# alexncoleman/WeaklySupervisedDL

Hardware: AMD Instinct MI355X
Metric: SegmentationModel train img/s at B=16 256x256 (higher is better)
Workload: dtype f32

## Files before the change

weaklysuperviseddl_amd/csrc/conv_igemm.hip:

```cpp
#include "common.h"

#include <type_traits>
#include <algorithm>
#include <cstdint>
#include <mutex>

typedef float f32x16 __attribute__((ext_vector_type(16)));

namespace {

constexpr int kThreads = 256;

struct ConvSrc {
    const float* x;
    const float* wt;
    const float* x_amax;
    int KH, KW, bh, ch, K, Cin;
    long long x_bs;
    unsigned x_bytes;
};

struct ConvP {
    const float* x;
    const float* wt;
    float* y;
    const float* scale;
    const float* shift;
    const float* res;
    int B, Cin, H, W, Cout, OH, OW, KH, KW;
    int ah, bh, ch, sh;
    int K;
    long long x_bs, y_bs, res_bs;
    int relu, accumulate;
    int P;
    unsigned x_bytes;
    int ksplit;
    float* slab;
    int ow0, own;
    int nb;
    int b_ow0[4], b_own[4], b_tile0[5];
    int grid_x;
    int xcd_py;
    int xcd_rowfast;
    int tile_img_major;
    const float* x_amax;
    float* y_amax;
    const uint8_t* acc_mask;
    const float* acc_base;
    int nsrc;
    ConvSrc src[3];
};

__device__ __forceinline__ float acc_prev(const ConvP& p, const float* ptr) {
    float o = *ptr;
    if (p.acc_mask) {
        const long long e = ptr - p.acc_base;
        if (!((p.acc_mask[e >> 3] >> (e & 7)) & 1)) o = 0.f;
    }
    return o;
}

template <int BM, int BN, int WM, bool ALIGNED>
__global__ __launch_bounds__(kThreads) void conv_igemm_kernel(ConvP p) {
    constexpr int BK = 16;
    constexpr int WN = 4 / WM;
    constexpr int MI = BM / WM / 32;
    constexpr int NI = BN / WN / 32;
    static_assert(MI >= 1 && NI >= 1 && MI * 32 * WM == BM && NI * 32 * WN == BN, "bad tile");
    constexpr int A_F4 = BK * BM / 4 / kThreads;
    constexpr int B_STEP = kThreads / BN;
    constexpr int B_PER = BK / B_STEP;

    __shared__ float As[2][BK * BM];
    __shared__ float Bs[2][BK * BN];
    __shared__ int vtaps[64];
    constexpr int kTab = ALIGNED ? 1 : 1024;
    __shared__ int ktab[kTab][2];
// ... 1149 lines not shown
    WSDL_LAUNCH_CHECK();
    return WSDL_OK;
}

wsdl::Opt g_conv_split{1};
wsdl::Opt g_conv_arith{1};
bool split_eligible(int rows, int kc, int T) {
    return g_conv_split && kc % 16 == 0 && T <= 9 && split_layout_bytes(g_conv_arith, (long long)T * kc, rows) < (1ll << 31);
}

wsdl::Opt g_xcd_map{1};
int choose_xcd_py(const ConvP& p, int gx, int gy) {
    if (!g_xcd_map || p.ksplit > 1 || ((long long)gx * gy) % 8 != 0) return 0;
    const double wb = (g_conv_arith ? 4.0 : 6.0) * (double)p.K * p.Cout, xb = 4.0 * (double)p.B * p.Cin * p.H * p.W;
    int best = 0;
    double best_cost = 0.0;
    for (int py = 1; py <= 8; py *= 2) {
        const int px = 8 / py;
        if (gy % py || gx % px) continue;
        if (g_xcd_map > 10 && py != g_xcd_map - 10) continue;
        const double cost = wb * px + xb * py;
        if (!best || cost < best_cost) { best = py; best_cost = cost; }
    }
    if (g_xcd_map == 1 && (best <= 1 || best_cost > 0.9 * (wb * 8 + xb))) return 0;
    return best;
}

template <int BM, int BN, int WM, int BK>
int launch_split(const ConvP& p_in, hipStream_t s, dim3 grid) {
    ConvP p = p_in;
    grid.z = p.ksplit > 1 ? p.ksplit : 1;
    p.xcd_py = choose_xcd_py(p, grid.x, grid.y);
    p.tile_img_major = 0;
    constexpr bool MF = BK == 32;
    WSDL_TRACE("split<%d,%d,%d> ar=%d %s ks=%d xcd_py=%d nb=%d grid=%ux%ux%u", BM, BN, BK, (int)g_conv_arith,
               (MF && g_conv_arith) ? "mfma16x16x32" : "mfma32x32x16", p.ksplit, p.xcd_py, p.nb, grid.x, grid.y, grid.z);
    if (g_conv_arith == 2)
        hipLaunchKernelGGL((conv_igemm_split_kernel<BM, BN, WM, BK, kThreads, 2, MF>), grid, dim3(kThreads), 0, s, p);
    else if (g_conv_arith)
        hipLaunchKernelGGL((conv_igemm_split_kernel<BM, BN, WM, BK, kThreads, 1, MF>), grid, dim3(kThreads), 0, s, p);
    else
        hipLaunchKernelGGL((conv_igemm_split_kernel<BM, BN, WM, BK, kThreads, 0>), grid, dim3(kThreads), 0, s, p);
    WSDL_LAUNCH_CHECK();
    return WSDL_OK;
}

wsdl::Opt g_conv_il{1};
int launch_split_256x128(const ConvP& p_in, hipStream_t s) {
    ConvP p = p_in;
    dim3 grid(p.grid_x > 0 ? p.grid_x : wsdl::cdiv(p.P, 128), wsdl::cdiv(p.Cout, 256), p.ksplit > 1 ? p.ksplit : 1);
    p.xcd_py = choose_xcd_py(p, grid.x, grid.y);
    p.xcd_rowfast = 0;
    p.tile_img_major = 0;
    if (p.nsrc > 0 && grid.y % 2 == 0 && ((long long)grid.x * grid.y) % 8 == 0) {
        int py = 4;
        while (py > 1 && (grid.y % py || grid.x % (8 / py))) py /= 2;
        if (grid.y % py == 0 && grid.x % (8 / py) == 0) {
            p.xcd_py = py;
            p.xcd_rowfast = 1;
        }
    }
    WSDL_TRACE("split<256,128,16> ar=%d il=%d nsrc=%d ks=%d xcd_py=%d rowfast=%d imgmajor=%d nb=%d grid=%ux%ux%u", (int)g_conv_arith,
               (int)(g_conv_arith == 1 && g_conv_il), p.nsrc, p.ksplit, p.xcd_py, p.xcd_rowfast, p.tile_img_major, p.nb, grid.x, grid.y, grid.z);
    if (p.nsrc > 0) {
        if (g_conv_arith == 2) hipLaunchKernelGGL((conv_igemm_split_kernel<256, 128, 4, 16, 512, 2, false, true>), grid, dim3(512), 0, s, p);
        else if (g_conv_arith && g_conv_il)
            hipLaunchKernelGGL((conv_igemm_split_kernel<256, 128, 4, 16, 512, 1, false, true, true>), grid, dim3(512), 0, s, p);
        else if (g_conv_arith) hipLaunchKernelGGL((conv_igemm_split_kernel<256, 128, 4, 16, 512, 1, false, true>), grid, dim3(512), 0, s, p);
        else hipLaunchKernelGGL((conv_igemm_split_kernel<256, 128, 4, 16, 512, 0, false, true>), grid, dim3(512), 0, s, p);
        WSDL_LAUNCH_CHECK();
        return WSDL_OK;
    }
    if (g_conv_arith == 2) hipLaunchKernelGGL((conv_igemm_split_kernel<256, 128, 4, 16, 512, 2>), grid, dim3(512), 0, s, p);
    else if (g_conv_arith && g_conv_il)
        hipLaunchKernelGGL((conv_igemm_split_kernel<256, 128, 4, 16, 512, 1, false, false, true>), grid, dim3(512), 0, s, p);
    else if (g_conv_arith) hipLaunchKernelGGL((conv_igemm_split_kernel<256, 128, 4, 16, 512, 1>), grid, dim3(512), 0, s, p);
    else hipLaunchKernelGGL((conv_igemm_split_kernel<256, 128, 4, 16, 512, 0>), grid, dim3(512), 0, s, p);
    WSDL_LAUNCH_CHECK();
    return WSDL_OK;
}

template <int BM, int BN, int WM>
int launch_cfg(const ConvP& p, hipStream_t s, bool aligned, bool split) {
    dim3 grid(p.grid_x > 0 ? p.grid_x : wsdl::cdiv(p.P, BN), wsdl::cdiv(p.Cout, BM));
    constexpr bool kSmallTile = BM * BN <= 128 * 64;
    if (split) {
        if constexpr (kSmallTile) {
            if (p.Cin % 32 == 0) {
                return launch_split<BM, BN, WM, 32>(p, s, grid);
            }
        }
        return launch_split<BM, BN, WM, 16>(p, s, grid);
    } else if (aligned) {
        if constexpr (kSmallTile) {
            if (p.Cin % 32 == 0) {
                return launch_fast<BM, BN, WM, 32>(p, s, grid);
// ... 387 lines not shown
            hipLaunchKernelGGL(wgrad_reduce_kernel, dim3(d.nblocks), dim3(256), 0, s, d.slab, d.dw, d.S, d.Cout, d.Cin, d.T, d.accumulate,
                               d.live);
            break;
    }
    WSDL_LAUNCH_CHECK();
    return WSDL_OK;
}

template <int BM, int BN, int WM>
int launch_wgrad_fast(const WgradP& p, hipStream_t s, int S) {
    dim3 grid(p.N / BN, p.Cout / BM, S);
    hipLaunchKernelGGL((conv_wgrad_fast_kernel<BM, BN, WM, 16>), grid, dim3(kThreads), 2 * (BM + BN) * 17 * sizeof(float), s, p);
    WSDL_LAUNCH_CHECK();
    return WSDL_OK;
}

}

extern "C" {

int wsdl_set_option(const char* name, int value) {
    WSDL_REQUIRE(name, "set_option: null name");
    static std::mutex mu;
    std::lock_guard<std::mutex> lock(mu);
    WSDL_REQUIRE(wsdl::g_plans_recording.load() == 0,
                 "set_option(%s): a launch plan is being recorded (its launches are chosen under ONE option set)", name);
    if (!strcmp(name, "tile_threshold")) { g_tile_threshold = value; return WSDL_OK; }
    if (!strcmp(name, "conv_split")) { g_conv_split = value != 0; return WSDL_OK; }
    if (!strcmp(name, "stem_kernel")) { g_stem_kernel = value != 0; return WSDL_OK; }
    if (!strcmp(name, "wgrad_direct")) { g_wgrad_direct = value; return WSDL_OK; }
    if (!strcmp(name, "wgrad_chan_scale")) { g_wgrad_chan_scale = value != 0; return WSDL_OK; }
    if (!strcmp(name, "wgrad_dyraw")) { g_wgrad_dyraw = value; return WSDL_OK; }
    if (!strcmp(name, "conv_il")) { g_conv_il = value != 0; return WSDL_OK; }
    if (!strcmp(name, "xcd_map")) { g_xcd_map = value; return WSDL_OK; }
    if (!strcmp(name, "ksplit_target")) { g_ksplit_target = value; return WSDL_OK; }
    if (!strcmp(name, "ksplit_max")) { g_ksplit_max = value; return WSDL_OK; }
    if (!strcmp(name, "ksplit_min_chunks")) { g_ksplit_min_chunks = value > 0 ? value : 1; return WSDL_OK; }
    if (!strcmp(name, "conv_arith")) {
        WSDL_REQUIRE(value >= 0 && value <= 2, "conv_arith: 0 (bf16x3), 1 (fp16x2), 2 (fp16x2, low piece at 2^11)");
        g_conv_arith = value;
        return WSDL_OK;
    }
    if (!strcmp(name, "range_sentinel")) { wsdl::g_range_sentinel = value != 0; return WSDL_OK; }
    if (!strcmp(name, "group_tps10")) { g_group_tps10 = value > 0 ? value : 45; return WSDL_OK; }
    if (!strcmp(name, "bn_resident")) { wsdl::g_bn_resident = value; return WSDL_OK; }
    if (!strcmp(name, "bn_wide_c")) { wsdl::g_bn_wide_c = value; return WSDL_OK; }
    if (!strcmp(name, "layercam_tail_mod")) {
        WSDL_REQUIRE(value >= 0 && value <= 32, "layercam_tail_mod: 0..32");
        wsdl::g_layercam_tail_mod = value;
        return WSDL_OK;
    }
    if (!strcmp(name, "wgrad_split")) { g_wgrad_split = value != 0; return WSDL_OK; }
    if (!strcmp(name, "wgrad_xcd")) { g_wgrad_xcd = value; return WSDL_OK; }
    if (!strcmp(name, "wgrad_min_tiles")) { g_wgrad_min_tiles = value > 0 ? value : 1; return WSDL_OK; }
    if (!strcmp(name, "wgrad_blocks")) { g_wgrad_blocks = value > 0 ? value : 768; return WSDL_OK; }
    wsdl::set_error("set_option: unknown option %s", name);
    return WSDL_EINVAL;
}

size_t wsdl_conv2d_weight_layout_bytes(int Cout, int Cin, int kh, int kw, int dgrad, int* is_plain) {
    const int T = kh * kw;
    const bool split = dgrad ? split_eligible(Cin, Cout, T) : split_eligible(Cout, Cin, T);
    if (is_plain) *is_plain = split ? 0 : 1;
    const size_t n = (size_t)Cout * Cin * T;
    return split ? (size_t)split_layout_bytes(g_conv_arith, (long long)T * (dgrad ? Cout : Cin), dgrad ? Cin : Cout) : n * 4;
}
// ... 159 lines not shown
        p.B = B; p.Cin = Cin; p.H = H; p.W = W; p.Cout = Cout; p.OH = H; p.OW = W; p.KH = p.KW = k[i];
        p.ah = 1; p.bh = dil[i]; p.ch = -pad; p.sh = 1;
        p.K = k[i] * k[i] * Cin;
        p.x_bs = xbs;
        p.y_bs = (y_bs && y_bs[i]) ? y_bs[i] : (long long)Cout * H * W;
        p.res_bs = p.y_bs;
        WSDL_REQUIRE(p.x_bs >= (long long)Cin * H * W && p.y_bs >= (long long)Cout * H * W, "conv2d_fwd_group: batch stride smaller than an image");
        p.P = B * H * W;
        p.x_bytes = (unsigned)(((long long)(B - 1) * p.x_bs + (long long)Cin * H * W) * 4);
        p.x_amax = x_amax;
        p.ow0 = 0; p.own = W; p.nb = 1;
        Band bands[8];
        int nb = 1;
        bands[0] = Band{0, W};
        nb = column_bands(W, W, p.ah, p.bh, p.ch, p.sh, p.KW, bands);
        int tiles = 0;
        for (int b = 0; b < nb && nb > 1; ++b) {
            p.b_ow0[b] = bands[b].ow0;
            p.b_own[b] = bands[b].own;
            p.b_tile0[b] = tiles;
            tiles += wsdl::cdiv((long long)B * H * bands[b].own, 128);
        }
        p.nb = nb;
        p.b_tile0[nb > 1 ? nb : 0] = tiles;
        const int gx = nb > 1 ? tiles : wsdl::cdiv(p.P, 128), gy = Cout / 256;
        const int ks = group_ksplit(group_max_taps(H, W, k[i], dil[i]));
        p.ksplit = ks;
        if (ks > 1) {
            p.slab = reinterpret_cast<float*>(wsp);
            wsp += wsdl::align_up((size_t)ks * Cout * p.P * sizeof(float), 256);
        }
        p.xcd_py = (start % 8 == 0) ? choose_xcd_py(p, gx, gy) : 0;
        p.tile_img_major = k[i] > 1;
        grp.start[j] = start;
        grp.gx[j] = gx;
        grp.gy[j] = gy;
        start += gx * gy * ks;
        const double f = 2.0 * p.P * (double)Cout * p.K;
        flops += f;
        if (wsdl::prof_enabled()) {
            for (int b = 0; b < nb; ++b) {
                ConvP q = p;
                q.ow0 = bands[b].ow0; q.own = bands[b].own; q.P = B * H * q.own;
                executed += f * ((double)q.own / W) * igemm_executed_fraction(q, 128);
            }
        }
        bytes += 4.0 * ((double)p.K * Cout + (double)p.P * Cout);
    }
    grp.start[n] = start;
    {
        int ns = 0;
        bool same = true;
        for (int j = 0; j < n; ++j) {
            ns += grp.p[j].ksplit;
            same = same && grp.gx[j] * grp.gy[j] == grp.gx[0] * grp.gy[0];
        }
        if (same && ns <= 8 && (8 % ns == 0)) {
            grp.ns = ns;
            int s = 0;
            for (int j = 0; j < n; ++j)
                for (int z = 0; z < grp.p[j].ksplit; ++z) {
                    grp.s_prob[s] = j;
                    grp.s_slice[s] = z;
                    ++s;
                }
            for (int j = 0; j < n; ++j) grp.p[j].xcd_py = 0;
        }
    }
    {
        wsdl::ProfScope prof(WSDL_PROF_SPLIT_GROUP, s, flops, wsdl::prof_enabled() ? executed : flops, bytes);
        WSDL_TRACE("group split<256,128,16> ar=%d il=%d problems=%d streams=%d ks=%d/%d/%d/%d workgroups=%d", (int)g_conv_arith,
                   (int)(g_conv_arith == 1 && g_conv_il), n, grp.ns, grp.p[0].ksplit, n > 1 ? grp.p[1].ksplit : 0,
                   n > 2 ? grp.p[2].ksplit : 0, n > 3 ? grp.p[3].ksplit : 0, start);
        if (g_conv_arith == 2)
            hipLaunchKernelGGL((conv_igemm_split_group_kernel<256, 128, 4, 16, 512, 2>), dim3(start), dim3(512), 0, s, grp);
        else if (g_conv_arith && g_conv_il)
            hipLaunchKernelGGL((conv_igemm_split_group_kernel<256, 128, 4, 16, 512, 1, false, true>), dim3(start), dim3(512), 0, s, grp);
        else if (g_conv_arith)
            hipLaunchKernelGGL((conv_igemm_split_group_kernel<256, 128, 4, 16, 512, 1>), dim3(start), dim3(512), 0, s, grp);
        else
            hipLaunchKernelGGL((conv_igemm_split_group_kernel<256, 128, 4, 16, 512, 0>), dim3(start), dim3(512), 0, s, grp);
        WSDL_LAUNCH_CHECK();
    }
    for (int j = 0; j < n; ++j) {
        const ConvP& p = grp.p[j];
        if (p.ksplit <= 1) continue;
        const long long total = (long long)p.Cout * p.P;
        const bool vec4 = p.y_bs % 4 == 0 && (reinterpret_cast<uintptr_t>(p.y) & 15) == 0;
        if (vec4)
            hipLaunchKernelGGL(conv_splitk_reduce_vec4_kernel, dim3((int)std::min<long long>((total / 4 + 255) / 256, 8192)),
                               dim3(256), 0, s, p);
        else
            hipLaunchKernelGGL(conv_splitk_reduce_kernel, dim3((int)std::min<long long>((total + 255) / 256, 4096)),
                               dim3(256), 0, s, p);
        WSDL_LAUNCH_CHECK();
    }
    return WSDL_OK;
}

int wsdl_conv2d_dgrad_multi_ok(int n, int B, int Cin, int H, int W, int Cout) {
    if (n < 2 || n > 4 || !g_conv_split) return 0;
    if (Cin % 256 != 0 || Cout % 16 != 0) return 0;
    if ((long long)wsdl::cdiv((long long)B * H * W, 128) * (Cin / 256) < 256) return 0;
    if ((long long)wsdl::cdiv((long long)B * H * W, 128) * wsdl::cdiv(Cin, 128) < g_tile_threshold) return 0;
    if (igemm_ksplit(B * H * W, Cin, Cout, 9, 1) != 1) return 0;
    if (((long long)(B - 1) * Cout * H * W + (long long)Cout * H * W) * 4 > (1ll << 31) - 4) return 0;
    return 1;
}

int wsdl_conv2d_dgrad_multi(int n, const float* const* dy, const void* const* wt_dgrad, const float* const* dy_amax,
                            const int* k, const int* dil, const long long* dy_bs, float* dx, int B, int Cin, int H, int W,
                            int Cout, int accumulate, wsdl_stream_t stream) {
    WSDL_REQUIRE(dy && wt_dgrad && dy_amax && k && dil && dx, "conv2d_dgrad_multi: null pointer");
    WSDL_REQUIRE(wsdl_conv2d_dgrad_multi_ok(n, B, Cin, H, W, Cout), "conv2d_dgrad_multi: geometry not supported (see "
                 "wsdl_conv2d_dgrad_multi_ok): %d sources, B %d, %d -> %d channels, %d x %d", n, B, Cin, Cout, H, W);
    ConvP p{};
    double flops = 0.0;
    for (int i = 0; i < n; ++i) {
        WSDL_REQUIRE(dy[i] && wt_dgrad[i], "conv2d_dgrad_multi: null source %d", i);
        WSDL_REQUIRE((k[i] == 1 || k[i] == 3) && dil[i] >= 1, "conv2d_dgrad_multi: source %d: 1x1 or 3x3, stride 1", i);
        WSDL_REQUIRE(split_eligible(Cin, Cout, k[i] * k[i]), "conv2d_dgrad_multi: source %d is not on the split kernels", i);
        WSDL_REQUIRE(!g_conv_arith || dy_amax[i], "conv2d_dgrad_multi: source %d: the fp16x2 kernels need dy_amax", i);
        const int pad = dil[i] * (k[i] - 1) / 2;
        const long long bs = (dy_bs && dy_bs[i]) ? dy_bs[i] : (long long)Cout * H * W;
        WSDL_REQUIRE(bs >= (long long)Cout * H * W, "conv2d_dgrad_multi: batch stride smaller than an image");
        const unsigned xbytes = (unsigned)(((long long)(B - 1) * bs + (long long)Cout * H * W) * 4);
        WSDL_REQUIRE(((long long)(B - 1) * bs + (long long)Cout * H * W) * 4 <= (1ll << 31) - 4, "conv2d_dgrad_multi: dY extent >= 2 GiB");
        flops += 2.0 * (double)B * H * W * (double)Cout * k[i] * k[i] * Cin;
        if (i == 0) {
            p.x = dy[0]; p.wt = static_cast<const float*>(wt_dgrad[0]); p.x_amax = dy_amax[0];
            p.KH = p.KW = k[0]; p.bh = -dil[0]; p.ch = pad; p.K = k[0] * k[0] * Cout; p.x_bs = bs; p.x_bytes = xbytes;
        } else {
            ConvSrc& c = p.src[i - 1];
            c.x = dy[i]; c.wt = static_cast<const float*>(wt_dgrad[i]); c.x_amax = dy_amax[i];
            c.KH = c.KW = k[i]; c.bh = -dil[i]; c.ch = pad; c.K = k[i] * k[i] * Cout; c.Cin = Cout; c.x_bs = bs; c.x_bytes = xbytes;
        }
    }
    p.nsrc = n - 1;
    p.y = dx;
    p.B = B; p.Cin = Cout; p.H = H; p.W = W; p.Cout = Cin; p.OH = H; p.OW = W;
    p.ah = 1; p.sh = 1;
    p.y_bs = (long long)Cin * H * W;
    p.res_bs = p.y_bs;
    p.relu = 0; p.accumulate = accumulate; p.P = B * H * W;
    p.acc_mask = nullptr; p.acc_base = dx;
    p.y_amax = nullptr;
    return launch_igemm(p, wsdl::as_stream(stream), flops, nullptr, 0);
}

int wsdl_conv2d_prep_weights_multi(const wsdl_prep_desc* desc, int n, int total_blocks, wsdl_stream_t stream) {
    WSDL_REQUIRE(desc && n > 0 && total_blocks > 0, "prep_weights_multi: bad arguments");
    WSDL_REQUIRE(g_conv_arith >= 1 && g_conv_split, "prep_weights_multi: only the fp16x2 split layouts");
    if (g_conv_arith == 2)
        hipLaunchKernelGGL(prep_weights_split_multi_kernel<2>, dim3(total_blocks), dim3(256), 0, wsdl::as_stream(stream), desc, n);
    else
        hipLaunchKernelGGL(prep_weights_split_multi_kernel<1>, dim3(total_blocks), dim3(256), 0, wsdl::as_stream(stream), desc, n);
    WSDL_LAUNCH_CHECK();
    return WSDL_OK;
}

size_t wsdl_conv2d_igemm_workspace(int B, int Cin, int H, int W, int Cout, int kh, int kw, int stride,
                                   int pad, int dil, int dgrad) {
    int OH, OW;
    if (check_geom(B, Cin, H, W, Cout, kh, kw, stride, pad, dil, &OH, &OW)) return 0;
    const int P = dgrad ? B * H * W : B * OH * OW, M = dgrad ? Cin : Cout, Kc = dgrad ? Cout : Cin;
    const int ks = igemm_ksplit(P, M, Kc, kh * kw, dil);
    return ks > 1 ? (size_t)ks * M * P * sizeof(float) : 0;
}

__global__ void channel_amax_kernel(const float* __restrict__ t, int B, int C, int HW, long long bs, float* __restrict__ out) {
    const int c = blockIdx.x;
// ... 515 lines not shown
```

weaklysuperviseddl_amd/csrc/conv_split.h:

```cpp
#pragma once

typedef __bf16 bf16x8 __attribute__((ext_vector_type(8)));
typedef __bf16 bf16x2 __attribute__((ext_vector_type(2)));
typedef _Float16 half8 __attribute__((ext_vector_type(8)));
typedef float f32x4 __attribute__((ext_vector_type(4)));

__device__ __forceinline__ void split3(float x0, float x1, unsigned& h, unsigned& m, unsigned& l) {
    f32x2 v = {x0, x1};
    h = __builtin_bit_cast(unsigned, __builtin_convertvector(v, bf16x2));
    f32x2 r = {x0 - __builtin_bit_cast(float, h << 16), x1 - __builtin_bit_cast(float, h & 0xffff0000u)};
    m = __builtin_bit_cast(unsigned, __builtin_convertvector(r, bf16x2));
    f32x2 s = {r[0] - __builtin_bit_cast(float, m << 16), r[1] - __builtin_bit_cast(float, m & 0xffff0000u)};
    l = __builtin_bit_cast(unsigned, __builtin_convertvector(s, bf16x2));
}

__device__ __forceinline__ void split2hs(float x0, float x1, unsigned& h, unsigned& l) {
    f32x2 v = {x0, x1};
    const half2v hv = __builtin_convertvector(v, half2v);
    h = __builtin_bit_cast(unsigned, hv);
    f32x2 r = {(x0 - (float)hv[0]) * 2048.f, (x1 - (float)hv[1]) * 2048.f};
    l = __builtin_bit_cast(unsigned, __builtin_convertvector(r, half2v));
}

template <int AR> struct SplitArith;
// ... 5 lines not shown
    }
};
template <> struct SplitArith<1> {
    static constexpr int NP = 2;
    using frag = half8;
    static __device__ __forceinline__ f32x16 mma(frag a, frag b, f32x16 c) {
        return __builtin_amdgcn_mfma_f32_32x32x16_f16(a, b, c, 0, 0, 0);
    }
};
template <> struct SplitArith<2> : SplitArith<1> {};
template <int AR, typename F>
__device__ __forceinline__ f32x16 split_products(const F (&a)[SplitArith<AR>::NP], const F (&b)[SplitArith<AR>::NP], f32x16 c) {
    using A = SplitArith<AR>;
    if constexpr (AR == 0) {
        c = A::mma(a[2], b[0], c);
        c = A::mma(a[0], b[2], c);
        c = A::mma(a[1], b[1], c);
        c = A::mma(a[1], b[0], c);
        c = A::mma(a[0], b[1], c);
        c = A::mma(a[0], b[0], c);
    } else {
        c = A::mma(a[1], b[0], c);
        c = A::mma(a[0], b[1], c);
        c = A::mma(a[0], b[0], c);
    }
    return c;
}

constexpr int split_k16_bytes(int AR) { return AR ? 64 : 96; }
__host__ __device__ constexpr long long split_layout_bytes(int AR, long long k_total, long long rows) {
    return (k_total / 16) * rows * split_k16_bytes(AR) + 16;
}

template <int BM, int BN, int WM, int BK, int NT, int AR, bool MF, bool MS, bool IL>
__device__ __forceinline__ void conv_igemm_split_body(const ConvP& p, const int bx_in, const int by_in, const int bz,
                                                      const int grid_x, const int grid_y) {
    static_assert(!MF || (AR >= 1 && BK == 32), "16x16x32 form: fp16x2, K chunk 32");
    using Ar = SplitArith<AR>;
    using frag = typename Ar::frag;
    constexpr int NP = Ar::NP;
    constexpr int K16B = split_k16_bytes(AR);
    constexpr int WN = (NT / 64) / WM;
    constexpr int MI = BM / WM / 32, NI = BN / WN / 32;
    static_assert(MI >= 1 && NI >= 1 && MI * 32 * WM == BM && NI * 32 * WN == BN, "bad tile");
    static_assert(BK == 16 || BK == 32, "K chunk");
    constexpr int KS = BK / 16;
    constexpr int ROW = MF ? 128 : KS * K16B + 16;
    constexpr int UPR = K16B / 16;
    constexpr int A_UPS = BM * UPR;
    constexpr int A_U = (KS * A_UPS + NT - 1) / NT;
    constexpr bool A_EXACT = A_U * NT == KS * A_UPS;
    constexpr int B_STEP = NT / BN;
    constexpr int B_PER = BK / B_STEP;
    static_assert(B_PER == 4 || B_PER == 8 || B_PER == 16 || B_PER == 32, "B tile");
    constexpr unsigned kOOB = 0x80000000u;

    __shared__ __attribute__((aligned(16))) unsigned char As[2][BM * ROW];
    __shared__ __attribute__((aligned(16))) unsigned char Bs[2][BN * ROW];
    __shared__ int vtaps[64];

    const int tid = threadIdx.x;
    const int lane = tid & 63, wid = tid >> 6;
    const int wm = wid / WN, wn = wid % WN;
    int bx = bx_in, by = by_in;
    if (p.xcd_py > 0) {
        const int gx = grid_x;
        const int L = by * gx + bx;
        const int xcd = L & 7, idx = L >> 3;
        const int py = p.xcd_py, px = 8 / py;
        const int lx = gx / px, ly = grid_y / py;
        if (p.xcd_rowfast) {
            bx = (xcd / py) * lx + idx / ly;
            by = (xcd % py) * ly + idx % ly;
        } else {
            bx = (xcd / py) * lx + idx % lx;
            by = (xcd % py) * ly + idx / lx;
        }
    }
    const int m0 = by * BM;
    int w_ow0 = p.ow0, w_own = p.own, w_tile0 = 0;
    if (p.nb > 1) {
        w_ow0 = p.b_ow0[0];
        w_own = p.b_own[0];
#pragma unroll
        for (int i = 1; i < 4; ++i)
            if (i < p.nb && bx >= p.b_tile0[i]) {
                w_ow0 = p.b_ow0[i];
                w_own = p.b_own[i];
                w_tile0 = p.b_tile0[i];
            }
    }
    const int W_P = p.nb > 1 ? p.B * p.OH * w_own : p.P;
// ... 68 lines not shown
#pragma unroll
                for (int i = 0; i < TMI; ++i)
#pragma unroll
                    for (int j = 0; j < TNI; ++j)
#pragma unroll
                        for (int r = 0; r < RT; ++r) {
                            acc[i][j][r] *= f;
                            if constexpr (LO) acc_lo[i][j][r] *= f;
                        }
            }
            e_units = ex + ew;
        }
    }
    const unsigned img_off = (unsigned)((long long)pb * s_x_bs) + (unsigned)(kr * B_PER * HW);

    auto tap_src = [&](int t, int& sp) {
        const int ti = t / s_KW, tj = t - ti * s_KW;
        const int nh = poh * p.ah + ti * s_bh + s_ch;
        const int nw = pow_ * p.ah + tj * s_bh + s_ch;
        bool ok = pix_ok && nh >= 0 && nw >= 0;
        int ih = nh, iw = nw;
        if (p.sh != 1) {
            ih = nh / p.sh;
            iw = nw / p.sh;
            ok = ok && (ih * p.sh == nh) && (iw * p.sh == nw);
        }
        ok = ok && ih < p.H && iw < p.W;
        sp = ih * p.W + iw;
        return ok;
    };

    const int T = s_KH * s_KW;
    const int cpt = s_Cin / BK;
    int nv = 0;
    for (int t = 0; t < T; ++t) {
        int sp;
        const bool ok = tap_src(t, sp);
        if (__syncthreads_or(ok)) {
            if (tid == 0) vtaps[nv] = t;
            ++nv;
        }
    }
    const int nq_all = nv * cpt;
    const int q0 = p.ksplit > 1 ? (int)((long long)nq_all * bz / p.ksplit) : 0;
    const int q1 = p.ksplit > 1 ? (int)((long long)nq_all * (bz + 1) / p.ksplit) : nq_all;
    const int nq = q1 - q0;
    __syncthreads();

    constexpr bool kRowMajorA = UPR == 4 && (A_UPS % 64) == 0;
    unsigned voff_a[A_U], lds_a[A_U];
#pragma unroll
    for (int e = 0; e < A_U; ++e) {
        const int u = tid + e * NT;
        const int ks = u / A_UPS, v = u - ks * A_UPS;
        const int j = v & 63;
        const int row = kRowMajorA ? (v >> 6) * 16 + (j & 7) + 8 * (j >> 5) : v / UPR;
        const int part = kRowMajorA ? (j >> 3) & 3 : v - row * UPR;
        voff_a[e] = (m0 + row < p.Cout && (A_EXACT || u < KS * A_UPS))
                        ? (unsigned)(ks * p.Cout * K16B + ((m0 + row) * UPR + part) * 16) : kOOB;
        if constexpr (MF)
            lds_a[e] = (unsigned)(row * ROW + (((4 * (part >> 1) + 2 * ks + (part & 1)) ^ (row & 7)) << 4));
        else
            lds_a[e] = (unsigned)(row * ROW + ks * K16B + part * 16);
    }

    u32x4 ra[A_U];
    unsigned rb[B_PER];
    int ld_vi = q0 / cpt, ld_c = q0 - (q0 / cpt) * cpt, ld_tap = 0;
    unsigned voff_b = kOOB;
    auto set_tap = [&](int vi) {
        ld_tap = __builtin_amdgcn_readfirstlane(vtaps[vi]);
        int sp;
        const bool ok = tap_src(ld_tap, sp);
        voff_b = ok ? (img_off + (unsigned)sp) * 4u : kOOB;
    };
    if (nq > 0) set_tap(ld_vi);

    auto load_next = [&]() {
        if (ld_c == cpt) {
            ld_c = 0;
            ++ld_vi;
            set_tap(ld_vi);
        }
        const int c16 = (ld_tap * s_Cin + ld_c * BK) / 16;
        const unsigned soff_a = (unsigned)(c16 * p.Cout * K16B);
#pragma unroll
        for (int e = 0; e < A_U; ++e) ra[e] = __builtin_amdgcn_raw_buffer_load_b128(rw, voff_a[e], soff_a, 0);
        const unsigned soff_b = (unsigned)(ld_c * BK * HW) * 4u;
#pragma unroll
        for (int e = 0; e < B_PER; ++e)
            rb[e] = __builtin_amdgcn_raw_buffer_load_b32(rx, voff_b, soff_b + (unsigned)(e * HW) * 4u, 0);
        ++ld_c;
    };
    auto store_tiles = [&](int buf) {
#pragma unroll
        for (int e = 0; e < A_U; ++e)
            if (A_EXACT || tid + e * NT < KS * A_UPS) *reinterpret_cast<u32x4*>(&As[buf][lds_a[e]]) = ra[e];
        unsigned pc[NP][B_PER / 2];
#pragma unroll
        for (int e = 0; e < B_PER / 2; ++e) {
            const float x0 = __builtin_bit_cast(float, rb[2 * e]), x1 = __builtin_bit_cast(float, rb[2 * e + 1]);
            if constexpr (AR == 0)
                split3(x0, x1, pc[0][e], pc[1][e], pc[2][e]);
            else if constexpr (AR == 1)
                split2h(x0 * xs, x1 * xs, pc[0][e], pc[1][e]);
            else
                split2hs(x0 * xs, x1 * xs, pc[0][e], pc[1][e]);
        }
        unsigned char* rowp = &Bs[buf][pl * ROW];
        if constexpr (MF) {
            static_assert(!MF || B_PER == 8 || B_PER == 16 || B_PER == 32, "a thread's run is whole k-groups");
#pragma unroll
            for (int g = 0; g < B_PER / 8; ++g) {
                const int kg = kr * (B_PER / 8) + g;
#pragma unroll
                for (int c = 0; c < NP; ++c)
                    *reinterpret_cast<u32x4*>(rowp + (((4 * c + kg) ^ (pl & 7)) << 4)) =
                        u32x4{pc[c][4 * g], pc[c][4 * g + 1], pc[c][4 * g + 2], pc[c][4 * g + 3]};
            }
        } else if constexpr (B_PER == 4) {
            const int k = kr * 4, off = (k / 16) * K16B + (k % 16) * 2;
#pragma unroll
            for (int c = 0; c < NP; ++c) *reinterpret_cast<u32x2*>(rowp + off + c * 32) = u32x2{pc[c][0], pc[c][1]};
        } else {
#pragma unroll
// ... 53 lines not shown
#pragma unroll
            for (int ks = 0; ks < KS; ++ks) {
                frag a[MI][NP], b[NI][NP];
#pragma unroll
                for (int i = 0; i < MI; ++i)
#pragma unroll
                    for (int c = 0; c < NP; ++c)
                        a[i][c] = *reinterpret_cast<const frag*>(Ab + i * 32 * ROW + ks * K16B + c * 32);
#pragma unroll
                for (int j = 0; j < NI; ++j)
#pragma unroll
                    for (int c = 0; c < NP; ++c)
                        b[j][c] = *reinterpret_cast<const frag*>(Bb + j * 32 * ROW + ks * K16B + c * 32);
#pragma unroll
                for (int i = 0; i < MI; ++i)
#pragma unroll
                    for (int j = 0; j < NI; ++j) {
                        if constexpr (!MF && LO) {
                            acc_lo[i][j] = Ar::mma(a[i][1], b[j][0], acc_lo[i][j]);
                            acc_lo[i][j] = Ar::mma(a[i][0], b[j][1], acc_lo[i][j]);
                            acc[i][j] = Ar::mma(a[i][0], b[j][0], acc[i][j]);
                        } else if constexpr (!MF) {
                            acc[i][j] = split_products<AR>(a[i], b[j], acc[i][j]);
                        }
                    }
            }
        }
    };
    int q_start = 0;
    if constexpr (IL) {
        static_assert(!IL || (!MF && KS == 1 && AR == 1), "interleaved loop: 32x32x16 form, K chunk 16, fp16x2");
        unsigned il_soff_a = 0, il_soff_b = 0;
        auto advance = [&]() {
            if (ld_c == cpt) {
                ld_c = 0;
                ++ld_vi;
                set_tap(ld_vi);
            }
            il_soff_a = (unsigned)(((ld_tap * s_Cin + ld_c * BK) / 16) * p.Cout * K16B);
            il_soff_b = (unsigned)(ld_c * BK * HW) * 4u;
            ++ld_c;
        };
        const unsigned fra = (unsigned)((wm * (MI * 32) + l31) * ROW + lh * 16), frb = (unsigned)((wn * (NI * 32) + l31) * ROW + lh * 16);
        int q = 0;
        if (nq > 2) advance();
        for (; q + 2 < nq; ++q) {
            const int cur = q & 1;
            frag a[MI][NP], b[NI][NP];
#pragma unroll
            for (int i = 0; i < MI; ++i)
#pragma unroll
                for (int c = 0; c < NP; ++c) a[i][c] = *reinterpret_cast<const frag*>(&As[cur][fra + i * 32 * ROW + c * 32]);
#pragma unroll
            for (int j = 0; j < NI; ++j)
#pragma unroll
                for (int c = 0; c < NP; ++c) b[j][c] = *reinterpret_cast<const frag*>(&Bs[cur][frb + j * 32 * ROW + c * 32]);
            store_tiles(cur ^ 1);
#pragma unroll
            for (int e = 0; e < A_U; ++e) ra[e] = __builtin_amdgcn_raw_buffer_load_b128(rw, voff_a[e], il_soff_a, 0);
#pragma unroll
            for (int e = 0; e < B_PER; ++e)
                rb[e] = __builtin_amdgcn_raw_buffer_load_b32(rx, voff_b, il_soff_b + (unsigned)(e * HW) * 4u, 0);
#pragma unroll
            for (int i = 0; i < MI; ++i)
#pragma unroll
                for (int j = 0; j < NI; ++j) acc[i][j] = split_products<AR>(a[i], b[j], acc[i][j]);
            __builtin_amdgcn_sched_group_barrier(0x100, (MI + NI) * NP, 0);
            __builtin_amdgcn_sched_group_barrier(0x002, 4, 0);
#pragma unroll
            for (int k = 0; k < MI * NI * 3; ++k) {
                __builtin_amdgcn_sched_group_barrier(0x008, 1, 0);
                __builtin_amdgcn_sched_group_barrier(0x002, 2, 0);
                if (k < 4) __builtin_amdgcn_sched_group_barrier(0x200, 1, 0);
                else if (k < 4 + A_U + B_PER) __builtin_amdgcn_sched_group_barrier(0x020, 1, 0);
// ... 40 lines not shown
    for (int j = 0; j < TNI; ++j) {
        const int opix = n0 + wn * (BN / WN) + j * TS + l31;
        if (opix >= W_P) continue;
        const int ob = opix / OHW;
        const int orr = opix - ob * OHW, ooh = orr / w_own;
        const int orp = ooh * p.OW + w_ow0 + (orr - ooh * w_own);
        float* yb = p.y + (long long)ob * p.y_bs + orp;
        const float* rbp = p.res ? p.res + (long long)ob * p.res_bs + orp : nullptr;
#pragma unroll
        for (int i = 0; i < TMI; ++i) {
#pragma unroll
            for (int r = 0; r < RT; ++r) {
                const int co = m0 + wm * (BM / WM) + i * TS + acc_row(r);
                if (co >= p.Cout) continue;
                float v = acc[i][j][r];
                if constexpr (LO) v = fmaf(acc_lo[i][j][r], 0x1p-11f, v);
                if constexpr (AR >= 1) v *= out_scale;
                if (p.scale) v *= p.scale[co];
                if (p.shift) v += p.shift[co];
                const long long off = (long long)co * OHOW;
                if (rbp) v += rbp[off];
                if (p.accumulate) v += acc_prev(p, yb + off);
                if (p.relu) v = fmaxf(v, 0.f);
                yb[off] = v;
                vmax = fmaxf(vmax, fabsf(v));
            }
        }
    }
    if (p.y_amax) publish_amax(vmax, p.y_amax);
}

template <int BM, int BN, int WM, int BK, int NT = kThreads, int AR = 1, bool MF = false, bool MS = false, bool IL = false>
__global__ __launch_bounds__(NT, NT == kThreads ? 2 : 1) void conv_igemm_split_kernel(ConvP p) {
    conv_igemm_split_body<BM, BN, WM, BK, NT, AR, MF, MS, IL>(p, blockIdx.x, blockIdx.y, blockIdx.z, gridDim.x, gridDim.y);
}

struct ConvGroup {
    int n;
    int start[5];
    int gx[4], gy[4];
    int ns;
    int s_prob[8], s_slice[8];
    ConvP p[4];
};
template <int BM, int BN, int WM, int BK, int NT = kThreads, int AR = 1, bool MF = false, bool IL = false>
__global__ __launch_bounds__(NT, NT == kThreads ? 2 : 1) void conv_igemm_split_group_kernel(ConvGroup grp) {
    const int L = blockIdx.x;
    if (grp.ns > 0) {
        const int s = L % grp.ns, r = L / grp.ns;
        const int g = grp.s_prob[s], gx = grp.gx[g], gy = grp.gy[g];
        conv_igemm_split_body<BM, BN, WM, BK, NT, AR, MF, false, IL>(grp.p[g], r % gx, r / gx, grp.s_slice[s], gx, gy);
        return;
    }
    int g = 0;
#pragma unroll
    for (int i = 1; i < 4; ++i)
        if (i < grp.n && L >= grp.start[i]) g = i;
    const int local = L - grp.start[g], gx = grp.gx[g], gy = grp.gy[g];
    const int plane = gx * gy, bz = local / plane, r = local - bz * plane;
    conv_igemm_split_body<BM, BN, WM, BK, NT, AR, MF, false, IL>(grp.p[g], r % gx, r / gx, bz, gx, gy);
}

__global__ void amax_kernel(const float* __restrict__ x, long long per, long long x_bs, long long total,
                            float* __restrict__ out) {
    float m = 0.f;
    if (x_bs == per && (per & 3) == 0 && (reinterpret_cast<unsigned long long>(x) & 15) == 0) {
        const float4* x4 = reinterpret_cast<const float4*>(x);
        for (long long i = blockIdx.x * (long long)blockDim.x + threadIdx.x; i < total / 4; i += (long long)gridDim.x * blockDim.x) {
            const float4 v = x4[i];
            m = fmaxf(fmaxf(m, fmaxf(fabsf(v.x), fabsf(v.y))), fmaxf(fabsf(v.z), fabsf(v.w)));
        }
    } else {
        for (long long i = blockIdx.x * (long long)blockDim.x + threadIdx.x; i < total; i += (long long)gridDim.x * blockDim.x) {
            const long long b = i / per;
            m = fmaxf(m, fabsf(x[b * x_bs + (i - b * per)]));
        }
    }
    publish_amax(m, out);
}

__global__ void multi_amax_kernel(const float* const* __restrict__ ptrs, const long long* __restrict__ counts,
                                  float* __restrict__ out) {
    const float* x = ptrs[blockIdx.y];
    const long long n = counts[blockIdx.y];
    float m = 0.f;
    if ((n & 3) == 0 && (reinterpret_cast<unsigned long long>(x) & 15) == 0) {
        const float4* x4 = reinterpret_cast<const float4*>(x);
        for (long long i = blockIdx.x * (long long)blockDim.x + threadIdx.x; i < n / 4; i += (long long)gridDim.x * blockDim.x)
            m = amax4(m, x4[i]);
    } else {
        for (long long i = blockIdx.x * (long long)blockDim.x + threadIdx.x; i < n; i += (long long)gridDim.x * blockDim.x)
            m = fmaxf(m, fabsf(x[i]));
    }
// ... 859 lines not shown
```

Baseline: 910.0.

## Reorder split-conv K loop to iterate taps inside channel chunks

Adds a tap-inner K ordering to the split implicit-GEMM conv kernel for grouped and multi-source dgrad launches. Per-tap input offsets are precomputed into shared memory and tap ids are packed into a register, so the K loop walks all valid taps for one channel chunk before moving on. K-split boundaries are placed on channel chunks. The aim is better cache reuse of the same input channel slab across taps and less per-tap offset recomputation, at the cost of extra shared memory, more template instantiations and a different accumulation order.

```diff
diff --git a/weaklysuperviseddl_amd/csrc/conv_igemm.hip b/weaklysuperviseddl_amd/csrc/conv_igemm.hip
--- a/weaklysuperviseddl_amd/csrc/conv_igemm.hip
+++ b/weaklysuperviseddl_amd/csrc/conv_igemm.hip
@@ -43,6 +43,7 @@
     int xcd_py;
     int xcd_rowfast;
     int tile_img_major;
+    int tap_inner;
     const float* x_amax;
     float* y_amax;
     const uint8_t* acc_mask;
@@ -1258,6 +1259,7 @@
     grid.z = p.ksplit > 1 ? p.ksplit : 1;
     p.xcd_py = choose_xcd_py(p, grid.x, grid.y);
     p.tile_img_major = 0;
+    p.tap_inner = 0;
     constexpr bool MF = BK == 32;
     WSDL_TRACE("split<%d,%d,%d> ar=%d %s ks=%d xcd_py=%d nb=%d grid=%ux%ux%u", BM, BN, BK, (int)g_conv_arith,
                (MF && g_conv_arith) ? "mfma16x16x32" : "mfma32x32x16", p.ksplit, p.xcd_py, p.nb, grid.x, grid.y, grid.z);
@@ -1272,12 +1274,14 @@
 }
 
 wsdl::Opt g_conv_il{1};
+wsdl::Opt g_conv_tap_inner{1};
 int launch_split_256x128(const ConvP& p_in, hipStream_t s) {
     ConvP p = p_in;
     dim3 grid(p.grid_x > 0 ? p.grid_x : wsdl::cdiv(p.P, 128), wsdl::cdiv(p.Cout, 256), p.ksplit > 1 ? p.ksplit : 1);
     p.xcd_py = choose_xcd_py(p, grid.x, grid.y);
     p.xcd_rowfast = 0;
     p.tile_img_major = 0;
+    if (p.nsrc == 0) p.tap_inner = 0;
     if (p.nsrc > 0 && grid.y % 2 == 0 && ((long long)grid.x * grid.y) % 8 == 0) {
         int py = 4;
         while (py > 1 && (grid.y % py || grid.x % (8 / py))) py /= 2;
@@ -1286,8 +1290,9 @@
             p.xcd_rowfast = 1;
         }
     }
-    WSDL_TRACE("split<256,128,16> ar=%d il=%d nsrc=%d ks=%d xcd_py=%d rowfast=%d imgmajor=%d nb=%d grid=%ux%ux%u", (int)g_conv_arith,
-               (int)(g_conv_arith == 1 && g_conv_il), p.nsrc, p.ksplit, p.xcd_py, p.xcd_rowfast, p.tile_img_major, p.nb, grid.x, grid.y, grid.z);
+    WSDL_TRACE("split<256,128,16> ar=%d il=%d nsrc=%d ks=%d xcd_py=%d rowfast=%d imgmajor=%d tap_inner=%d nb=%d grid=%ux%ux%u", (int)g_conv_arith,
+               (int)(g_conv_arith == 1 && g_conv_il), p.nsrc, p.ksplit, p.xcd_py, p.xcd_rowfast, p.tile_img_major, p.tap_inner, p.nb,
+               grid.x, grid.y, grid.z);
     if (p.nsrc > 0) {
         if (g_conv_arith == 2) hipLaunchKernelGGL((conv_igemm_split_kernel<256, 128, 4, 16, 512, 2, false, true>), grid, dim3(512), 0, s, p);
         else if (g_conv_arith && g_conv_il)
@@ -1741,6 +1746,7 @@
     if (!strcmp(name, "wgrad_chan_scale")) { g_wgrad_chan_scale = value != 0; return WSDL_OK; }
     if (!strcmp(name, "wgrad_dyraw")) { g_wgrad_dyraw = value; return WSDL_OK; }
     if (!strcmp(name, "conv_il")) { g_conv_il = value != 0; return WSDL_OK; }
+    if (!strcmp(name, "conv_tap_inner")) { g_conv_tap_inner = value != 0; return WSDL_OK; }
     if (!strcmp(name, "xcd_map")) { g_xcd_map = value; return WSDL_OK; }
     if (!strcmp(name, "ksplit_target")) { g_ksplit_target = value; return WSDL_OK; }
     if (!strcmp(name, "ksplit_max")) { g_ksplit_max = value; return WSDL_OK; }
@@ -1966,6 +1972,7 @@
         }
         p.xcd_py = (start % 8 == 0) ? choose_xcd_py(p, gx, gy) : 0;
         p.tile_img_major = k[i] > 1;
+        p.tap_inner = g_conv_tap_inner && group_max_taps(H, W, k[i], dil[i]) > 1;
         grp.start[j] = start;
         grp.gx[j] = gx;
         grp.gy[j] = gy;
@@ -2003,9 +2010,11 @@
     }
     {
         wsdl::ProfScope prof(WSDL_PROF_SPLIT_GROUP, s, flops, wsdl::prof_enabled() ? executed : flops, bytes);
-        WSDL_TRACE("group split<256,128,16> ar=%d il=%d problems=%d streams=%d ks=%d/%d/%d/%d workgroups=%d", (int)g_conv_arith,
+        int any_tap_inner = 0;
+        for (int j = 0; j < n; ++j) any_tap_inner |= grp.p[j].tap_inner;
+        WSDL_TRACE("group split<256,128,16> ar=%d il=%d problems=%d streams=%d ks=%d/%d/%d/%d tap_inner=%d workgroups=%d", (int)g_conv_arith,
                    (int)(g_conv_arith == 1 && g_conv_il), n, grp.ns, grp.p[0].ksplit, n > 1 ? grp.p[1].ksplit : 0,
-                   n > 2 ? grp.p[2].ksplit : 0, n > 3 ? grp.p[3].ksplit : 0, start);
+                   n > 2 ? grp.p[2].ksplit : 0, n > 3 ? grp.p[3].ksplit : 0, any_tap_inner, start);
         if (g_conv_arith == 2)
             hipLaunchKernelGGL((conv_igemm_split_group_kernel<256, 128, 4, 16, 512, 2>), dim3(start), dim3(512), 0, s, grp);
         else if (g_conv_arith && g_conv_il)
@@ -2050,6 +2059,7 @@
                  "wsdl_conv2d_dgrad_multi_ok): %d sources, B %d, %d -> %d channels, %d x %d", n, B, Cin, Cout, H, W);
     ConvP p{};
     double flops = 0.0;
+    int live_taps = 1;
     for (int i = 0; i < n; ++i) {
         WSDL_REQUIRE(dy[i] && wt_dgrad[i], "conv2d_dgrad_multi: null source %d", i);
         WSDL_REQUIRE((k[i] == 1 || k[i] == 3) && dil[i] >= 1, "conv2d_dgrad_multi: source %d: 1x1 or 3x3, stride 1", i);
@@ -2061,6 +2071,7 @@
         const unsigned xbytes = (unsigned)(((long long)(B - 1) * bs + (long long)Cout * H * W) * 4);
         WSDL_REQUIRE(((long long)(B - 1) * bs + (long long)Cout * H * W) * 4 <= (1ll << 31) - 4, "conv2d_dgrad_multi: dY extent >= 2 GiB");
         flops += 2.0 * (double)B * H * W * (double)Cout * k[i] * k[i] * Cin;
+        live_taps = std::max(live_taps, group_max_taps(H, W, k[i], dil[i]));
         if (i == 0) {
             p.x = dy[0]; p.wt = static_cast<const float*>(wt_dgrad[0]); p.x_amax = dy_amax[0];
             p.KH = p.KW = k[0]; p.bh = -dil[0]; p.ch = pad; p.K = k[0] * k[0] * Cout; p.x_bs = bs; p.x_bytes = xbytes;
@@ -2071,6 +2082,7 @@
         }
     }
     p.nsrc = n - 1;
+    p.tap_inner = g_conv_tap_inner && live_taps > 1;
     p.y = dx;
     p.B = B; p.Cin = Cout; p.H = H; p.W = W; p.Cout = Cin; p.OH = H; p.OW = W;
     p.ah = 1; p.sh = 1;
diff --git a/weaklysuperviseddl_amd/csrc/conv_split.h b/weaklysuperviseddl_amd/csrc/conv_split.h
--- a/weaklysuperviseddl_amd/csrc/conv_split.h
+++ b/weaklysuperviseddl_amd/csrc/conv_split.h
@@ -61,7 +61,7 @@
     return (k_total / 16) * rows * split_k16_bytes(AR) + 16;
 }
 
-template <int BM, int BN, int WM, int BK, int NT, int AR, bool MF, bool MS, bool IL>
+template <int BM, int BN, int WM, int BK, int NT, int AR, bool MF, bool MS, bool IL, bool TI = false>
 __device__ __forceinline__ void conv_igemm_split_body(const ConvP& p, const int bx_in, const int by_in, const int bz,
                                                       const int grid_x, const int grid_y) {
     static_assert(!MF || (AR >= 1 && BK == 32), "16x16x32 form: fp16x2, K chunk 32");
@@ -87,6 +87,8 @@
     __shared__ __attribute__((aligned(16))) unsigned char As[2][BM * ROW];
     __shared__ __attribute__((aligned(16))) unsigned char Bs[2][BN * ROW];
     __shared__ int vtaps[64];
+    constexpr int kMaxTaps = 9;
+    __shared__ unsigned tapoff[TI ? kMaxTaps * BN : 1];
 
     const int tid = threadIdx.x;
     const int lane = tid & 63, wid = tid >> 6;
@@ -221,18 +223,38 @@
 
     const int T = s_KH * s_KW;
     const int cpt = s_Cin / BK;
+    const bool tap_inner = TI && p.tap_inner && T <= kMaxTaps;
+    unsigned tp_lo = 0, tp_hi = 0;
     int nv = 0;
     for (int t = 0; t < T; ++t) {
         int sp;
         const bool ok = tap_src(t, sp);
         if (__syncthreads_or(ok)) {
             if (tid == 0) vtaps[nv] = t;
+            if constexpr (TI) {
+                if (tap_inner) {
+                    if (kr == 0) tapoff[nv * BN + pl] = ok ? (unsigned)sp * 4u : kOOB;
+                    if (nv < 8) tp_lo |= (unsigned)t << (4 * nv);
+                    else tp_hi |= (unsigned)t << (4 * (nv - 8));
+                }
+            }
             ++nv;
         }
     }
+    if constexpr (TI) {
+        tp_lo = __builtin_amdgcn_readfirstlane(tp_lo);
+        tp_hi = __builtin_amdgcn_readfirstlane(tp_hi);
+    }
+    const unsigned long long tap_ids = ((unsigned long long)tp_hi << 32) | tp_lo;
     const int nq_all = nv * cpt;
-    const int q0 = p.ksplit > 1 ? (int)((long long)nq_all * bz / p.ksplit) : 0;
-    const int q1 = p.ksplit > 1 ? (int)((long long)nq_all * (bz + 1) / p.ksplit) : nq_all;
+    int q0 = p.ksplit > 1 ? (int)((long long)nq_all * bz / p.ksplit) : 0;
+    int q1 = p.ksplit > 1 ? (int)((long long)nq_all * (bz + 1) / p.ksplit) : nq_all;
+    int c_first = 0;
+    if (tap_inner && p.ksplit > 1) {
+        c_first = (int)((long long)cpt * bz / p.ksplit);
+        q0 = c_first * nv;
+        q1 = (int)((long long)cpt * (bz + 1) / p.ksplit) * nv;
+    }
     const int nq = q1 - q0;
     __syncthreads();
 
@@ -255,7 +277,7 @@
 
     u32x4 ra[A_U];
     unsigned rb[B_PER];
-    int ld_vi = q0 / cpt, ld_c = q0 - (q0 / cpt) * cpt, ld_tap = 0;
+    int ld_vi = tap_inner ? 0 : q0 / cpt, ld_c = tap_inner ? c_first : q0 - (q0 / cpt) * cpt, ld_tap = 0;
     unsigned voff_b = kOOB;
     auto set_tap = [&](int vi) {
         ld_tap = __builtin_amdgcn_readfirstlane(vtaps[vi]);
@@ -263,23 +285,37 @@
         const bool ok = tap_src(ld_tap, sp);
         voff_b = ok ? (img_off + (unsigned)sp) * 4u : kOOB;
     };
-    if (nq > 0) set_tap(ld_vi);
-
-    auto load_next = [&]() {
+    if (nq > 0 && !tap_inner) set_tap(ld_vi);
+    auto next_chunk = [&]() {
+        if constexpr (TI) {
+            if (tap_inner) {
+                const bool wrap = ld_vi == nv;
+                ld_vi = wrap ? 0 : ld_vi;
+                ld_c += wrap ? 1 : 0;
+                ld_tap = (int)(tap_ids >> (4 * ld_vi)) & 15;
+                voff_b = tapoff[ld_vi * BN + pl] + img_off * 4u;
+                ++ld_vi;
+                return ld_c;
+            }
+        }
         if (ld_c == cpt) {
             ld_c = 0;
             ++ld_vi;
             set_tap(ld_vi);
         }
-        const int c16 = (ld_tap * s_Cin + ld_c * BK) / 16;
+        return ld_c++;
+    };
+
+    auto load_next = [&]() {
+        const int c = next_chunk();
+        const int c16 = (ld_tap * s_Cin + c * BK) / 16;
         const unsigned soff_a = (unsigned)(c16 * p.Cout * K16B);
 #pragma unroll
         for (int e = 0; e < A_U; ++e) ra[e] = __builtin_amdgcn_raw_buffer_load_b128(rw, voff_a[e], soff_a, 0);
-        const unsigned soff_b = (unsigned)(ld_c * BK * HW) * 4u;
+        const unsigned soff_b = (unsigned)(c * BK * HW) * 4u;
 #pragma unroll
         for (int e = 0; e < B_PER; ++e)
             rb[e] = __builtin_amdgcn_raw_buffer_load_b32(rx, voff_b, soff_b + (unsigned)(e * HW) * 4u, 0);
-        ++ld_c;
     };
     auto store_tiles = [&](int buf) {
 #pragma unroll
@@ -399,14 +435,9 @@
         static_assert(!IL || (!MF && KS == 1 && AR == 1), "interleaved loop: 32x32x16 form, K chunk 16, fp16x2");
         unsigned il_soff_a = 0, il_soff_b = 0;
         auto advance = [&]() {
-            if (ld_c == cpt) {
-                ld_c = 0;
-                ++ld_vi;
-                set_tap(ld_vi);
-            }
-            il_soff_a = (unsigned)(((ld_tap * s_Cin + ld_c * BK) / 16) * p.Cout * K16B);
-            il_soff_b = (unsigned)(ld_c * BK * HW) * 4u;
-            ++ld_c;
+            const int c = next_chunk();
+            il_soff_a = (unsigned)(((ld_tap * s_Cin + c * BK) / 16) * p.Cout * K16B);
+            il_soff_b = (unsigned)(c * BK * HW) * 4u;
         };
         const unsigned fra = (unsigned)((wm * (MI * 32) + l31) * ROW + lh * 16), frb = (unsigned)((wn * (NI * 32) + l31) * ROW + lh * 16);
         int q = 0;
@@ -513,7 +544,7 @@
 
 template <int BM, int BN, int WM, int BK, int NT = kThreads, int AR = 1, bool MF = false, bool MS = false, bool IL = false>
 __global__ __launch_bounds__(NT, NT == kThreads ? 2 : 1) void conv_igemm_split_kernel(ConvP p) {
-    conv_igemm_split_body<BM, BN, WM, BK, NT, AR, MF, MS, IL>(p, blockIdx.x, blockIdx.y, blockIdx.z, gridDim.x, gridDim.y);
+    conv_igemm_split_body<BM, BN, WM, BK, NT, AR, MF, MS, IL, MS>(p, blockIdx.x, blockIdx.y, blockIdx.z, gridDim.x, gridDim.y);
 }
 
 struct ConvGroup {
@@ -530,7 +561,7 @@
     if (grp.ns > 0) {
         const int s = L % grp.ns, r = L / grp.ns;
         const int g = grp.s_prob[s], gx = grp.gx[g], gy = grp.gy[g];
-        conv_igemm_split_body<BM, BN, WM, BK, NT, AR, MF, false, IL>(grp.p[g], r % gx, r / gx, grp.s_slice[s], gx, gy);
+        conv_igemm_split_body<BM, BN, WM, BK, NT, AR, MF, false, IL, true>(grp.p[g], r % gx, r / gx, grp.s_slice[s], gx, gy);
         return;
     }
     int g = 0;
@@ -539,7 +570,7 @@
         if (i < grp.n && L >= grp.start[i]) g = i;
     const int local = L - grp.start[g], gx = grp.gx[g], gy = grp.gy[g];
     const int plane = gx * gy, bz = local / plane, r = local - bz * plane;
-    conv_igemm_split_body<BM, BN, WM, BK, NT, AR, MF, false, IL>(grp.p[g], r % gx, r / gx, bz, gx, gy);
+    conv_igemm_split_body<BM, BN, WM, BK, NT, AR, MF, false, IL, true>(grp.p[g], r % gx, r / gx, bz, gx, gy);
 }
 
 __global__ void amax_kernel(const float* __restrict__ x, long long per, long long x_bs, long long total,
```

After: 915.1, median of 6. No clear change (+0.6%).
